# esologic/GANce

Measured on AMD Instinct MI355X. Metric: synthesized frames/sec at 1024x1024 config-f, higher is better.
Workload: dtype f32 (bf16x3 split operands, 6 terms, fp32 accumulate)

## Files before the change

gance_amd/csrc/upfir_split.hip:

```cpp

#include <hip/hip_runtime.h>

#include <algorithm>
#include <cstring>
#include <type_traits>

#include "kernels.h"

#ifndef GANCE_UPFIRS_ABLATE
#define GANCE_UPFIRS_ABLATE 0
#endif

namespace gance {

namespace {

typedef float f32x4 __attribute__((ext_vector_type(4)));
typedef float f32x2 __attribute__((ext_vector_type(2)));
typedef unsigned u32x4 __attribute__((ext_vector_type(4)));
typedef unsigned u32x2 __attribute__((ext_vector_type(2)));
typedef __bf16 bf16x8 __attribute__((ext_vector_type(8)));
typedef __bf16 bf16x2 __attribute__((ext_vector_type(2)));
typedef __attribute__((address_space(3))) void* lds_ptr_t;

constexpr int kBM = 16;
constexpr int kKC = 32;
constexpr int kSW = 64;
constexpr int kTH = 8;
constexpr int kRows = kTH + 1;
constexpr int kPlanes = 12;
constexpr int kPlaneStride = 80;
constexpr int kSlotUnits = kPlanes * kPlaneStride;
constexpr int kRing = 3;
constexpr int kHaloCols = 4;
constexpr int kHaloUnits = kRows * kHaloCols * kPlanes;
constexpr int kHaloTasks = kRows * kHaloCols * 4;
constexpr int kWeave = 2;
constexpr int kMinSegRows = 16;
constexpr int kDepth = 6;
constexpr int kCarryRows = 3;
constexpr int kPassCh = 4;
constexpr int kPassRows = 8;
constexpr float kSqrt2f = 1.4142135623730951f;
static_assert((2 * kRows) % kDepth == 0 && kDepth + 2 < kRows && kRows % kRing == 0, "ring slots and staging registers rotate with the unrolled rows of a chunk pair");

template <int NT>
struct Geo {
    static constexpr int kSW = 64 / NT;
    static constexpr int kBMB = kBM * NT;
    static constexpr int kTC = kSW / 16;
    static constexpr int kPW = 4 / NT;
    static constexpr int kTW = 2 * kSW + 4;
    static constexpr int kCG = kSW / 2;
    static constexpr int kRG = 64 / NT / kCG;
    static constexpr int kFR = kPassRows / kRG;
    static constexpr int kWin = kFR + 3;
    static constexpr int kCarryFloats = kBMB * kCarryRows * kTW;
    static constexpr int kStageFloats = kPassCh * NT * kPassRows * kTW;
    static constexpr int kNzPieces = 2 * kPassRows * 2 * kSW / 256;
    static constexpr int kWUnits = NT == 1 ? 27 * 64 : 0;
};

constexpr size_t kRingBytes = (size_t)kRing * kSlotUnits * 16;
constexpr size_t kHaloBytes = (size_t)2 * kHaloUnits * 16;
template <int NT>
constexpr size_t lds_bytes(int cin) {
    using G = Geo<NT>;
    return kRingBytes + kHaloBytes + (size_t)G::kWUnits * 16 +
           sizeof(float) * ((size_t)G::kStageFloats + G::kNzPieces * 256 + G::kCarryFloats + cin + 3 * G::kBMB);
}

__host__ __device__ constexpr int tap_cls(int t) { return t < 4 ? 0 : (t < 6 ? 1 : (t < 8 ? 2 : 3)); }
__host__ __device__ constexpr int tap_dy(int t) { return (t == 2 || t == 3 || t == 5) ? 1 : 0; }
__host__ __device__ constexpr int tap_dx(int t) { return (t == 1 || t == 3 || t == 7) ? 1 : 0; }

__device__ __forceinline__ void lds_barrier() {
    asm volatile("s_waitcnt lgkmcnt(0)" ::: "memory");
    __builtin_amdgcn_s_barrier();
    asm volatile("" ::: "memory");
}

__device__ __forceinline__ int fresh_lane() {
    int l;
    asm volatile("v_mbcnt_lo_u32_b32 %0, -1, 0\n\tv_mbcnt_hi_u32_b32 %0, -1, %0" : "=v"(l));
    return l;
}

__device__ __forceinline__ int ring_column(int P) {
    return ((P >> 2) & 3) | ((((P >> 4) ^ P) & 1) << 2) | (((P >> 1) & 1) << 3) | ((P & 1) << 4) | (P & 32);
}
constexpr int kEdgeColumn = 64;

__device__ __forceinline__ void split_pair(float a, float b, unsigned& p0, unsigned& p1, unsigned& p2) {
    auto pack = [](float lo, float hi) { return __builtin_bit_cast(unsigned, __builtin_convertvector(f32x2{lo, hi}, bf16x2)); };
    p0 = pack(a, b);
    const float ra = a - __builtin_bit_cast(float, p0 << 16), rb = b - __builtin_bit_cast(float, p0 & 0xffff0000u);
    p1 = pack(ra, rb);
    const float sa = ra - __builtin_bit_cast(float, p1 << 16), sb = rb - __builtin_bit_cast(float, p1 & 0xffff0000u);
    p2 = pack(sa, sb);
}

__device__ __forceinline__ void split_unit(const unsigned (&raw)[8], u32x4 (&part)[3]) {
    unsigned w[3][4];
    if (GANCE_UPFIRS_ABLATE & 1) {
#pragma unroll
        for (int q = 0; q < 3; ++q) part[q] = u32x4{raw[q], raw[q + 1], raw[q + 2], raw[q + 3]};
        return;
    }
#pragma unroll
    for (int e = 0; e < 4; ++e) split_pair(__builtin_bit_cast(float, raw[2 * e]), __builtin_bit_cast(float, raw[2 * e + 1]), w[0][e], w[1][e], w[2][e]);
#pragma unroll
    for (int q = 0; q < 3; ++q) part[q] = u32x4{w[q][0], w[q][1], w[q][2], w[q][3]};
}

}

template <int NT, bool kPre, bool kNoise>
__device__ __forceinline__ void upfirs_body(const UpFirArgs& p) {
    using G = Geo<NT>;
    constexpr int kSW = G::kSW, kBMB = G::kBMB, kTC = G::kTC, kPW = G::kPW, kTW = G::kTW, kCG = G::kCG, kRG = G::kRG, kFR = G::kFR,
                  kWin = G::kWin, kCarryFloats = G::kCarryFloats, kStageFloats = G::kStageFloats, kNzPieces = G::kNzPieces;
    extern __shared__ __attribute__((aligned(16))) unsigned char smem_raw[];
    u32x4* const ring = reinterpret_cast<u32x4*>(smem_raw);
    u32x4* const halo = ring + kRing * kSlotUnits;
    u32x4* const w_lds = halo + 2 * kHaloUnits;
    float* const stage = reinterpret_cast<float*>(w_lds + G::kWUnits);
    float* const nz_lds = stage + kStageFloats;
    float* const carry = nz_lds + kNzPieces * 256;
    float* const s_lds = carry + kCarryFloats;
    float* const d_lds = s_lds + (kPre ? 0 : p.Cin);
    float* const b_lds = d_lds + kBMB;
    float* const sn_lds = b_lds + kBMB;

    const int tid = threadIdx.x;
    const int wave = __builtin_amdgcn_readfirstlane(tid >> 6);
    const int lane = tid & 63;
    const int n16 = lane & 15, kg = lane >> 4;
    const int ct = NT == 1 ? 0 : wave / kTC, tc = NT == 1 ? wave : wave % kTC;

    int id;
    {
        const int v = blockIdx.x, nwg = p.total_blocks;
        const int q = nwg >> 3, r = nwg & 7, xcd = v & 7;
        id = (xcd < r ? xcd * (q + 1) : r * (q + 1) + (xcd - r) * q) + (v >> 3);
    }
    const int m_tile = id % p.m_tiles;
    id /= p.m_tiles;
    const int strip = id % p.strips;
    id /= p.strips;
    const int seg = id % p.segs;
    const int b = id / p.segs;
    const int m0 = m_tile * kBMB;
    const int X0 = strip * kSW;
    const int H = p.H, W = p.W;
    const int Hp = H + 2, Wp = W + 8;
    const int HpWp4 = Hp * Wp * 4;
    const int chunks = p.Cin / kKC;
    const int steps = H / kTH;
    const int s_begin = seg * (p.rows_per_seg / kTH), s_end = s_begin + p.rows_per_seg / kTH;
    const int s_first = seg > 0 ? s_begin - 1 : s_begin;

    const __amdgpu_buffer_rsrc_t x_rsrc =
        __builtin_amdgcn_make_buffer_rsrc((void*)(p.x + (size_t)b * p.x_b_stride), 0, p.Cin * Hp * Wp * 4, 0x00020000);
    const __amdgpu_buffer_rsrc_t w_rsrc = __builtin_amdgcn_make_buffer_rsrc(
        (void*)(reinterpret_cast<const unsigned char*>(p.w) + (size_t)(m_tile * NT + ct) * chunks * 27 * 1024), 0, chunks * 27 * 1024, 0x00020000);

    const int st_pair = lane >> 4, st_g = lane & 15;
    u32x4* const ring_w = ring + wave * kPlaneStride + ring_column(4 * st_g + st_pair);
    unsigned* const ring_wn = reinterpret_cast<unsigned*>(ring + wave * kPlaneStride + ring_column(NT == 2 ? 2 * st_g + (st_pair & 1) : st_g)) +
                              (NT == 2 ? 2 * (st_pair >> 1) : st_pair);
    const int m_pos = 16 * tc + n16;
    const u32x4* const ring_r0 = ring + kg * kPlaneStride + ring_column(m_pos);
    const u32x4* const ring_r1 = ring + kg * kPlaneStride + (m_pos > 0 ? ring_column(m_pos - 1) : kEdgeColumn);
    const bool edge_copy = wave == 3 && lane < kPlanes;
    const int e_unit = lane % kPlanes;
    u32x4* const ring_e = ring + (e_unit >> 2) * 4 * kPlaneStride + (e_unit & 3) * kPlaneStride + (edge_copy ? kEdgeColumn : 66 + wave);
    const u32x4* const halo_e = halo + e_unit;
    const u32x4* const halo_r = halo + ((n16 & 7) * kHaloCols + 2 * (n16 >> 3)) * kPlanes + kg;
    const u32x4* const halo_f = halo + ((kRows - 1) * kHaloCols + 2 * (n16 >> 3)) * kPlanes + kg;
    const int st_voff = (2 * st_pair * Hp * Wp + X0 + 4 + kPW * st_g) * 4;
    unsigned st[kDepth][8];
    auto stage_load = [&](unsigned(&dst)[8], int chunk, int brow, bool in_loop = false) {
        if ((GANCE_UPFIRS_ABLATE & 4) && in_loop) return;
        const int soff = ((chunk * kKC + wave * 8) * Hp + brow) * Wp * 4;
#pragma unroll
        for (int e = 0; e < 2; ++e) {
            if constexpr (kPW == 4) {
                const u32x4 q4 = __builtin_amdgcn_raw_buffer_load_b128(x_rsrc, st_voff, soff + e * HpWp4, 0);
#pragma unroll
                for (int c = 0; c < 4; ++c) dst[2 * c + e] = q4[c];
            } else if constexpr (kPW == 2) {
                const u32x2 q2 = __builtin_amdgcn_raw_buffer_load_b64(x_rsrc, st_voff, soff + e * HpWp4, 0);
                dst[e] = q2[0];
                dst[2 + e] = q2[1];
            } else {
                dst[e] = __builtin_amdgcn_raw_buffer_load_b32(x_rsrc, st_voff, soff + e * HpWp4, 0);
            }
        }
    };
    auto scale_pair = [&](unsigned(&raw)[8], int chunk) {
        if constexpr (!kPre) {
            const f32x2 s2 = *reinterpret_cast<const f32x2*>(s_lds + chunk * kKC + 8 * wave + 2 * st_pair);
#pragma unroll
            for (int c = 0; c < kPW; ++c) {
                raw[2 * c] = __builtin_bit_cast(unsigned, __builtin_bit_cast(float, raw[2 * c]) * s2[0]);
                raw[2 * c + 1] = __builtin_bit_cast(unsigned, __builtin_bit_cast(float, raw[2 * c + 1]) * s2[1]);
            }
        }
    };
    auto transpose_rows = [](u32x4& u) {
        auto a02 = __builtin_amdgcn_permlane32_swap(u[0], u[2], false, false);
        auto a13 = __builtin_amdgcn_permlane32_swap(u[1], u[3], false, false);
        auto b01 = __builtin_amdgcn_permlane16_swap(a02[0], a13[0], false, false);
        auto b23 = __builtin_amdgcn_permlane16_swap(a02[1], a13[1], false, false);
        u = u32x4{b01[0], b01[1], b23[0], b23[1]};
    };
    auto scale8 = [&](unsigned(&raw)[8], int chunk, int group) {
        if constexpr (!kPre) {
            const f32x4 s0 = *reinterpret_cast<const f32x4*>(s_lds + chunk * kKC + group * 8);
            const f32x4 s1 = *reinterpret_cast<const f32x4*>(s_lds + chunk * kKC + group * 8 + 4);
#pragma unroll
            for (int e = 0; e < 4; ++e) {
                raw[e] = __builtin_bit_cast(unsigned, __builtin_bit_cast(float, raw[e]) * s0[e]);
                raw[4 + e] = __builtin_bit_cast(unsigned, __builtin_bit_cast(float, raw[4 + e]) * s1[e]);
            }
        }
    };
    auto stage_store = [&](unsigned(&raw)[8], int slot, int chunk) {
        scale_pair(raw, chunk);
        if constexpr (NT == 1) {
            u32x4 part[3];
            split_unit(raw, part);
#pragma unroll
            for (int q = 0; q < 3; ++q) transpose_rows(part[q]);
#pragma unroll
            for (int q = 0; q < 3; ++q)
                if (!(GANCE_UPFIRS_ABLATE & 16)) ring_w[slot * kSlotUnits + q * 4 * kPlaneStride] = part[q];
        } else {
            unsigned w[3][kPW];
#pragma unroll
            for (int c = 0; c < kPW; ++c) split_pair(__builtin_bit_cast(float, raw[2 * c]), __builtin_bit_cast(float, raw[2 * c + 1]), w[0][c], w[1][c], w[2][c]);
#pragma unroll
            for (int q = 0; q < 3; ++q) {
                unsigned* const dst = ring_wn + 4 * (slot * kSlotUnits + q * 4 * kPlaneStride);
                if constexpr (NT == 2) {
                    const auto s = __builtin_amdgcn_permlane16_swap(w[q][0], w[q][1], false, false);
                    *reinterpret_cast<u32x2*>(dst) = u32x2{s[0], s[1]};
                } else {
                    *dst = w[q][0];
                }
            }
        }
    };
    auto edge_store = [&](int slot, int hbuf, int hrow) { if (!(GANCE_UPFIRS_ABLATE & 64)) ring_e[slot * kSlotUnits] = halo_e[hbuf * kHaloUnits + (hrow * kHaloCols + 1) * kPlanes]; };
    const int h_task = tid < kHaloTasks ? tid : tid - kHaloTasks;
    const int h_col = h_task & 3, h_kg = (h_task >> 2) & 3, h_row = h_task >> 4;
    const int h_voff = ((h_kg * 8 * Hp + h_row) * Wp + X0 + 2 + (h_col & 1) + (h_col >> 1) * (kSW + 1)) * 4;
    u32x4* const halo_w = halo + (h_row * kHaloCols + h_col) * kPlanes + h_kg;
    unsigned hraw[8];
    auto halo_load = [&](int step, int chunk) {
        const int soff = (chunk * kKC * Hp + kTH * step) * Wp * 4;
#pragma unroll
        for (int e = 0; e < 8; ++e) hraw[e] = __builtin_amdgcn_raw_buffer_load_b32(x_rsrc, h_voff, soff + e * HpWp4, 0);
    };
    auto halo_store = [&](int chunk, int buf) {
        scale8(hraw, chunk, h_kg);
        u32x4 part[3];
        split_unit(hraw, part);
#pragma unroll
        for (int q = 0; q < 3; ++q) halo_w[buf * kHaloUnits + q * 4] = part[q];
    };

    u32x4 A[9][3];
    const int a_voff = lane * 16;
    auto weights_dma = [&](int chunk) {
#pragma unroll
        for (int k = 0; k < 7; ++k)
            if (k < 6 || wave < 3)
                __builtin_amdgcn_raw_ptr_buffer_load_lds(w_rsrc, (lds_ptr_t)(w_lds + (wave + 4 * k) * 64), 16, lane * 16, (chunk * 27 + wave + 4 * k) * 1024, 0, 0);
    };
    const u32x4* const w_r = w_lds + lane;
    auto read_a3 = [&](int t, u32x4(&dst)[3]) {
#pragma unroll
        for (int q = 0; q < 3; ++q) dst[q] = w_r[(t * 3 + q) * 64];
    };
    auto load_a3 = [&](int chunk, int t, u32x4(&dst)[3]) {
#pragma unroll
        for (int q = 0; q < 3; ++q) dst[q] = __builtin_amdgcn_raw_buffer_load_b128(w_rsrc, a_voff, (chunk * 27 + t * 3 + q) * 1024, 0);
    };

    u32x4 Bf[2][2][3];
    auto load_b = [&](int slot, u32x4(&dst)[2][3]) {
#pragma unroll
        for (int q = 0; q < 3; ++q) {
            dst[0][q] = ring_r0[slot * kSlotUnits + q * 4 * kPlaneStride];
            dst[1][q] = ring_r1[slot * kSlotUnits + q * 4 * kPlaneStride];
        }
    };

    stage_load(st[0], 0, kTH * s_first + 0);
    stage_load(st[1], 0, kTH * s_first + 1);
    load_a3(0, 0, A[0]);
    halo_load(s_first, 0);
    if constexpr (!kPre)
        for (int i = tid; i < p.Cin; i += 256) s_lds[i] = p.s[(size_t)b * p.s_stride + i];
    if (tid < kBMB) {
        d_lds[tid] = p.d[(size_t)b * p.d_stride + m0 + tid];
        b_lds[tid] = p.bias[m0 + tid];
        sn_lds[tid] = p.s_next != nullptr ? p.s_next[(size_t)b * p.s_stride + m0 + tid] : 1.0f;
    }
    for (int i = tid; i < kCarryFloats; i += 256) carry[i] = 0.f;
    if constexpr (NT > 1)
        for (int i = tid; i < kPassCh * NT * kPassRows; i += 256) stage[i * kTW] = stage[i * kTW + 2 * kSW + 2] = stage[i * kTW + 2 * kSW + 3] = 0.f;
#pragma unroll
    for (int t = 1; t < 9; ++t) load_a3(0, t, A[t]);
    if constexpr (!kPre) lds_barrier();
    stage_store(st[0], 0, 0);
    stage_store(st[1], 1, 0);
    halo_store(0, 0);
#pragma unroll
    for (int r = 2; r < 2 + kDepth; ++r) stage_load(st[r % kDepth], 0, kTH * s_first + r);
    lds_barrier();
    edge_store(0, 0, 0);
    edge_store(1, 0, 1);
    lds_barrier();
    load_b(0, Bf[0]);

    const int OW = 2 * W, OWp = OW + 8;
    const long long oplane = (long long)(2 * H + 2) * OWp;
    const __amdgpu_buffer_rsrc_t o_rsrc = __builtin_amdgcn_make_buffer_rsrc(
        (void*)(p.out + ((size_t)b * p.Cout + m0) * oplane - 2 * OWp), 0, 0x7fffffff, 0x00020000);
    const __amdgpu_buffer_rsrc_t nz_rsrc = __builtin_amdgcn_make_buffer_rsrc(
        (void*)(kNoise ? p.noise + (size_t)b * p.noise_b_stride : nullptr), 0, kNoise ? (2 * H) * (2 * W) * 4 : 0, 0x00020000);
    const float ns2 = p.noise_strength * kSqrt2f;

    constexpr int kTerms[6][2] = {{2, 0}, {0, 2}, {1, 1}, {1, 0}, {0, 1}, {0, 0}};
    constexpr int kTapTurn[9] = {0, 4, 6, 8, 2, 5, 1, 7, 3};

#pragma unroll 1
    for (int si = s_first; si < s_end; ++si) {
        const int y0 = kTH * si;
        const bool last_step = si + 1 == steps;
        const bool priming = si < s_begin;
        f32x4 acc[kTH][4];
#pragma unroll
        for (int r = 0; r < kTH; ++r)
#pragma unroll
            for (int c = 0; c < 4; ++c) acc[r][c] = f32x4{0.f, 0.f, 0.f, 0.f};
        f32x4 accf[2] = {f32x4{0.f, 0.f, 0.f, 0.f}, f32x4{0.f, 0.f, 0.f, 0.f}};
        f32x4 acch[NT == 1 ? 1 : 2] = {}, acchf = f32x4{0.f, 0.f, 0.f, 0.f};

        auto run_chunk = [&](auto parity, const int chunk) {
            constexpr int ab = decltype(parity)::value;
            const int n_chunk = chunk + 1 < chunks ? chunk + 1 : 0;
            const int n_step = chunk + 1 < chunks ? si : (last_step ? si : si + 1);
#pragma unroll
            for (int j = 0; j < kRows; ++j) {
                const int cur = (j + ab) & 1;
                if (NT == 1 && j == 0) weights_dma(n_chunk);
                if (j == 0) halo_load(n_step, n_chunk);
                if (j == 4) halo_store(n_chunk, ab ^ 1);
                load_b((j + 1) % kRing, Bf[cur ^ 1]);
                edge_store((j + 2) % kRing, j + 2 < kRows ? ab : ab ^ 1, (j + 2) % kRows);
                stage_store(st[(kRows * ab + j + 2) % kDepth], (j + 2) % kRing, j + 2 < kRows ? chunk : n_chunk);
                stage_load(st[(kRows * ab + j + 2) % kDepth], j + 2 + kDepth < kRows ? chunk : n_chunk, kTH * (j + 2 + kDepth < kRows ? si : n_step) + (j + 2 + kDepth) % kRows, true);
                if (j + 1 < kRows) {
#pragma unroll
                    for (int term = 0; term < ((GANCE_UPFIRS_ABLATE & 8) ? 0 : 6); ++term)
#pragma unroll
                        for (int k = 0; k < 9; ++k) {
                            const int t = kTapTurn[k];
                            const int row = tap_dy(t) ? j : j - 1;
                            if (row < 0 || row >= kTH) continue;
                            acc[row][tap_cls(t)] = __builtin_amdgcn_mfma_f32_16x16x32_bf16(
                                __builtin_bit_cast(bf16x8, A[t][kTerms[term][1]]), __builtin_bit_cast(bf16x8, Bf[cur][tap_dx(t)][kTerms[term][0]]),
                                acc[row][tap_cls(t)], 0, 0, 0);
                        }
#pragma unroll
                    for (int i = 0; i < 54; ++i) {
                        if (i >= (j == 0 ? 18 : 54)) break;
                        __builtin_amdgcn_sched_group_barrier(0x008, 1, 0);
                        __builtin_amdgcn_sched_group_barrier(0x092, kWeave, 0);
                    }
                } else {
                    constexpr int kOrder[9] = {2, 3, 5, 0, 1, 4, 6, 7, 8};
#pragma unroll
                    for (int i = 0; i < 9; ++i) {
                        const int t = kOrder[i];
                        if (!tap_dy(t)) {
#pragma unroll
                            for (int term = 0; term < 6; ++term)
                                acc[kTH - 1][tap_cls(t)] = __builtin_amdgcn_mfma_f32_16x16x32_bf16(
                                    __builtin_bit_cast(bf16x8, A[t][kTerms[term][1]]), __builtin_bit_cast(bf16x8, Bf[cur][tap_dx(t)][kTerms[term][0]]),
                                    acc[kTH - 1][tap_cls(t)], 0, 0, 0);
                        } else if (last_step) {
#pragma unroll
                            for (int term = 0; term < 6; ++term)
                                accf[tap_cls(t)] = __builtin_amdgcn_mfma_f32_16x16x32_bf16(
                                    __builtin_bit_cast(bf16x8, A[t][kTerms[term][1]]), __builtin_bit_cast(bf16x8, Bf[cur][tap_dx(t)][kTerms[term][0]]),
                                    accf[tap_cls(t)], 0, 0, 0);
                        }
                        const int hc = NT == 1 ? 0 : tap_cls(t) >> 1;
                        const bool halo_mine = NT == 1 ? wave == tap_cls(t) : (tap_dx(t) && (tap_cls(t) & 1) == 0 && (kTC == 1 || tc == hc));
                        if (halo_mine && !(GANCE_UPFIRS_ABLATE & 64)) {
                            u32x4 hf[3];
#pragma unroll
                            for (int q = 0; q < 3; ++q) hf[q] = halo_r[ab * kHaloUnits + ((1 - tap_dy(t)) * kHaloCols + 1 - tap_dx(t)) * kPlanes + q * 4];
#pragma unroll
                            for (int term = 0; term < 6; ++term)
                                acch[hc] = __builtin_amdgcn_mfma_f32_16x16x32_bf16(__builtin_bit_cast(bf16x8, A[t][kTerms[term][1]]),
                                                                                    __builtin_bit_cast(bf16x8, hf[kTerms[term][0]]), acch[hc], 0, 0, 0);
                            if (last_step && tap_dy(t)) {
#pragma unroll
                                for (int q = 0; q < 3; ++q) hf[q] = halo_f[ab * kHaloUnits + (1 - tap_dx(t)) * kPlanes + q * 4];
#pragma unroll
                                for (int term = 0; term < 6; ++term)
                                    acchf = __builtin_amdgcn_mfma_f32_16x16x32_bf16(__builtin_bit_cast(bf16x8, A[t][kTerms[term][1]]),
                                                                                    __builtin_bit_cast(bf16x8, hf[kTerms[term][0]]), acchf, 0, 0, 0);
                            }
                        }
                        if constexpr (NT == 1) read_a3(t, A[t]);
                        else load_a3(n_chunk, t, A[t]);
                    }
                }
                if (NT == 1 && j == kRows - 2) asm volatile("s_waitcnt vmcnt(24)" ::: "memory");
                if (!(GANCE_UPFIRS_ABLATE & 32)) lds_barrier();
            }
        };
#pragma unroll 1
        for (int chunk = 0; chunk < chunks; chunk += 2) {
            run_chunk(std::integral_constant<int, 0>{}, chunk);
            run_chunk(std::integral_constant<int, 1>{}, chunk + 1);
        }

        const int elane = fresh_lane();
        const int en16 = elane & 15, eq4 = elane >> 4;
        const int dump_base = (4 * ct + eq4) * (kPassRows * kTW) + 32 * tc + 2 * en16 + 1;
        const int hpy = wave >> 1, hpx = wave & 1;
        const int fsub = NT == 1 ? 0 : elane / (64 / NT), flane = NT == 1 ? elane : elane % (64 / NT);
        const int fc = NT == 1 ? wave : wave * NT + fsub;
        const int fch = NT == 1 ? fc : 16 * (fc >> 2) + (fc & 3);
        const int cg = flane % kCG;
        const int rg = flane / kCG;
        const int o_voff = (int)((fch * oplane + (long long)(kFR * rg) * OWp + 4 * cg) * 4);

        auto run_passes = [&](auto flush_tag) {
            constexpr bool kFlush = decltype(flush_tag)::value;
            const int ys = kFlush ? H : y0;
            if (kNoise) {
#pragma unroll
                for (int i = 0; i < (kNzPieces + 3) / 4; ++i) {
                    if (kNzPieces % 4 != 0 && wave + 4 * i >= kNzPieces) break;
                    const int f = (wave + 4 * i) * 256 + 4 * elane;
                    const int row = f / (2 * kSW), col = f % (2 * kSW);
                    __builtin_amdgcn_raw_ptr_buffer_load_lds(nz_rsrc, (lds_ptr_t)(nz_lds + (wave + 4 * i) * 256), 16,
                                                             ((2 * ys - 2 + row) * OW + 2 * X0 + col) * 4, 0, 0, 0);
                }
                asm volatile("s_waitcnt vmcnt(0)" ::: "memory");
            }
            constexpr int kRowPasses = kFlush ? 1 : 2;
#pragma unroll
            for (int rw = 0; rw < kRowPasses; ++rw) {
                const int oy0 = 2 * (ys + 4 * rw) - 2;
                const int r_lo = max(0, -oy0);
                const int r_hi = priming ? 0 : min(kPassRows, 2 * H - oy0);
#pragma unroll
                for (int g = 0; g < 4; ++g) {
                    if constexpr (kFlush) {
#pragma unroll
                        for (int c = 0; c < 4; ++c) stage[dump_base + (c >> 1) * kTW + (c & 1)] = c < 2 ? accf[c][g] : 0.f;
                        if constexpr (NT == 1) {
                            if (en16 == 0 || en16 == 8) {
                                const int side = en16 >> 3;
                                if (hpy == 0 && (side == 1 || hpx == 1)) stage[eq4 * (kPassRows * kTW) + (side ? 2 * kSW + 1 + hpx : 0)] = acchf[g];
                                if (hpy == 1 && (side == 1 || hpx == 1)) stage[eq4 * (kPassRows * kTW) + kTW + (side ? 2 * kSW + 1 + hpx : 0)] = 0.f;
                            }
                        } else if (en16 == 8 && tc == 0) {
                            stage[(4 * ct + eq4) * (kPassRows * kTW) + 2 * kSW + 1] = acchf[g];
                            stage[(4 * ct + eq4) * (kPassRows * kTW) + kTW + 2 * kSW + 1] = 0.f;
                        }
                    } else {
#pragma unroll
                        for (int r4 = 0; r4 < 4; ++r4)
#pragma unroll
                            for (int c = 0; c < 4; ++c) stage[dump_base + (2 * r4 + (c >> 1)) * kTW + (c & 1)] = acc[4 * rw + r4][c][g];
                        const int row = en16 & 7, side = en16 >> 3;
                        if constexpr (NT == 1) {
                            if ((side == 1 || hpx == 1) && row / 4 == rw)
                                stage[eq4 * (kPassRows * kTW) + (2 * (row % 4) + hpy) * kTW + (side ? 2 * kSW + 1 + hpx : 0)] = acch[0][g];
                        } else if (side == 1 && row / 4 == rw) {
#pragma unroll
                            for (int h = 0; h < 2; ++h)
                                if (kTC == 1 || tc == h) stage[(4 * ct + eq4) * (kPassRows * kTW) + (2 * (row % 4) + h) * kTW + 2 * kSW + 1] = acch[h][g];
                        }
                    }
                    lds_barrier();

                    const int ch = 4 * g + fch;
                    const float dsc = d_lds[ch] * kSqrt2f;
                    const float kh0 = 0.25f * dsc, kh1 = 0.75f * dsc;
                    const float bias2 = b_lds[ch] * kSqrt2f;
                    const float lr6 = 0.6f * sn_lds[ch], lr4 = 0.4f * sn_lds[ch];
                    const float* const win_lo = carry + ch * (kCarryRows * kTW) + (kFR * rg) * kTW + 4 * cg;
                    const float* const win_hi = stage + fc * (kPassRows * kTW) + (kFR * rg - kCarryRows) * kTW + 4 * cg;
                    f32x4 ta[kWin], tb[kWin];
#pragma unroll
                    for (int i = 0; i < kWin; ++i) {
                        const float* const rowp = (i < kCarryRows && kFR * rg + i < kCarryRows ? win_lo : win_hi) + i * kTW;
                        ta[i] = *reinterpret_cast<const f32x4*>(rowp);
                        tb[i] = *reinterpret_cast<const f32x4*>(rowp + 4);
                    }
                    {
                        const int o_soff = (int)((4 * g * oplane + (long long)(oy0 + 3) * OWp + 2 * X0 + 4) * 4);
#pragma unroll
                        for (int r = 0; r < kFR; ++r) {
                            const int rr = kFR * rg + r;
                            if (rr >= r_lo && rr < r_hi) {
                                f32x2 tv[4];
#pragma unroll
                                for (int c2 = 0; c2 < 4; ++c2) {
                                    auto pair = [&](int i) { return c2 < 2 ? f32x2{ta[i][2 * c2], ta[i][2 * c2 + 1]} : f32x2{tb[i][2 * c2 - 4], tb[i][2 * c2 - 3]}; };
                                    tv[c2] = 0.25f * pair(r) + 0.75f * pair(r + 1) + 0.75f * pair(r + 2) + 0.25f * pair(r + 3);
                                }
                                const float t[7] = {tv[0][0], tv[0][1], tv[1][0], tv[1][1], tv[2][0], tv[2][1], tv[3][0]};
                                f32x4 v;
#pragma unroll
                                for (int o = 0; o < 4; ++o) v[o] = fmaf(kh0, t[o + 3], fmaf(kh1, t[o + 2], fmaf(kh1, t[o + 1], fmaf(kh0, t[o], bias2))));
                                if (kNoise) v += ns2 * *reinterpret_cast<const f32x4*>(nz_lds + (kPassRows * rw + rr) * (2 * kSW) + 4 * cg);
#pragma unroll
                                for (int o = 0; o < 4; ++o) v[o] = fmaf(lr6, v[o], lr4 * __builtin_fabsf(v[o]));
                                if (!(GANCE_UPFIRS_ABLATE & 128)) __builtin_amdgcn_raw_buffer_store_b128(__builtin_bit_cast(u32x4, v), o_rsrc, o_voff, o_soff + r * OWp * 4, 0);
                                else asm volatile("" ::"v"(v));
                            }
                        }
                    }
                    lds_barrier();
                    if (!kFlush && rg == kRG - 1) {
                        float* const carry_w = carry + ch * (kCarryRows * kTW) + 4 * cg;
#pragma unroll
                        for (int i = 0; i < 3; ++i) {
                            *reinterpret_cast<f32x4*>(carry_w + i * kTW) = ta[kWin - 3 + i];
                            if (cg == kCG - 1) *reinterpret_cast<f32x4*>(carry_w + i * kTW + 4) = tb[kWin - 3 + i];
                        }
                    }
                }
            }
        };
        if (GANCE_UPFIRS_ABLATE & 2) {
            float sum = acch[0][0] + acchf[0] + accf[0][0] + accf[1][0];
#pragma unroll
            for (int r = 0; r < kTH; ++r)
#pragma unroll
                for (int c = 0; c < 4; ++c) sum += acc[r][c][0] + acc[r][c][3];
            if (sum == 12345.678f) p.out[tid] = sum;
            continue;
        }
        run_passes(std::false_type{});
        if (last_step) {
            lds_barrier();
            run_passes(std::true_type{});
        }
    }
}

bool upfirs_supported(int cin, int cout, int H, int W) {
    return H == W && W % kSW == 0 && H % kTH == 0 && cin % (2 * kKC) == 0 && cout % kBM == 0 && cin <= 512;
}

bool upfirs_narrow_supported(int cin, int cout, int H, int W) {
    return H == W && (W == 32 || W == 16) && H % kTH == 0 && cin % (2 * kKC) == 0 && cout % (kBM * (kSW / W)) == 0 && cin <= 512;
}

size_t upfirs_weight_floats(int cin, int cout) { return (size_t)(cout / kBM) * (cin / kKC) * 27 * 256; }

static unsigned short bf16_rne_host(float x) {
    unsigned u;
    std::memcpy(&u, &x, 4);
    u += 0x7fffu + ((u >> 16) & 1u);
    return (unsigned short)(u >> 16);
}
static float bf16_value_host(unsigned short h) {
    const unsigned u = (unsigned)h << 16;
    float f;
    std::memcpy(&f, &u, 4);
    return f;
}

void upfirs_arrange_weights(const float* w_in, int cin, int cout, const int* up_tap_weight, float* w_out) {
    unsigned short* const out = reinterpret_cast<unsigned short*>(w_out);
    const int m_tiles = cout / kBM, chunks = cin / kKC;
    for (int mt = 0; mt < m_tiles; ++mt)
        for (int ch = 0; ch < chunks; ++ch)
            for (int t = 0; t < 9; ++t)
                for (int k = 0; k < kKC; ++k)
                    for (int m = 0; m < kBM; ++m) {
                        const int channel = 4 * (m & 3) + (m >> 2);
                        const float v = w_in[((size_t)up_tap_weight[t] * cin + ch * kKC + k) * cout + mt * kBM + channel];
                        unsigned short part[3];
                        part[0] = bf16_rne_host(v);
                        const float r1 = v - bf16_value_host(part[0]);
                        part[1] = bf16_rne_host(r1);
                        part[2] = bf16_rne_host(r1 - bf16_value_host(part[1]));
                        for (int q = 0; q < 3; ++q)
                            out[((((((size_t)mt * chunks + ch) * 9 + t) * 3 + q) * 4 + k / 8) * 16 + m) * 8 + k % 8] = part[q];
                    }
}

void upfirs_plan(int B, int cout, int H, int W, int num_cus, UpFirArgs* a) {
    a->step_rows = kTH;
    if (W < kSW) {
        a->m_tiles = cout / (kBM * (kSW / W));
        a->strips = 1;
        a->segs = 1;
        a->rows_per_seg = H;
        a->total_blocks = B * a->m_tiles;
        return;
    }
    a->m_tiles = cout / kBM;
    a->strips = W / kSW;
    int segs = 1;
    const int base = B * a->m_tiles * a->strips;
    long long best = (long long)((base + num_cus - 1) / num_cus) * H;
    for (int n = 2; H / n >= kMinSegRows && (H / n) % kTH == 0 && base * (n / 2) < num_cus; n *= 2) {
        const long long cost = (long long)((base * n + num_cus - 1) / num_cus) * (H / n + kTH);
        if (cost < best) best = cost, segs = n;
    }
    a->segs = segs;
    a->rows_per_seg = H / segs;
    a->total_blocks = base * segs;
}

__global__ __launch_bounds__(256, 1) void upfirs_fused_kernel(const UpFirArgs p) { upfirs_body<1, false, false>(p); }
__global__ __launch_bounds__(256, 1) void upfirs_fused_noise_kernel(const UpFirArgs p) { upfirs_body<1, false, true>(p); }
__global__ __launch_bounds__(256, 1) void upfirs_fused_pre_kernel(const UpFirArgs p) { upfirs_body<1, true, false>(p); }
__global__ __launch_bounds__(256, 1) void upfirs_fused_pre_noise_kernel(const UpFirArgs p) { upfirs_body<1, true, true>(p); }
__global__ __launch_bounds__(256, 1) void upfirs_w32_fused_kernel(const UpFirArgs p) { upfirs_body<2, false, false>(p); }
__global__ __launch_bounds__(256, 1) void upfirs_w32_fused_noise_kernel(const UpFirArgs p) { upfirs_body<2, false, true>(p); }
__global__ __launch_bounds__(256, 1) void upfirs_w32_fused_pre_kernel(const UpFirArgs p) { upfirs_body<2, true, false>(p); }
__global__ __launch_bounds__(256, 1) void upfirs_w32_fused_pre_noise_kernel(const UpFirArgs p) { upfirs_body<2, true, true>(p); }
__global__ __launch_bounds__(256, 1) void upfirs_w16_fused_kernel(const UpFirArgs p) { upfirs_body<4, false, false>(p); }
__global__ __launch_bounds__(256, 1) void upfirs_w16_fused_noise_kernel(const UpFirArgs p) { upfirs_body<4, false, true>(p); }
__global__ __launch_bounds__(256, 1) void upfirs_w16_fused_pre_kernel(const UpFirArgs p) { upfirs_body<4, true, false>(p); }
__global__ __launch_bounds__(256, 1) void upfirs_w16_fused_pre_noise_kernel(const UpFirArgs p) { upfirs_body<4, true, true>(p); }

hipError_t launch_upfir_split(const UpFirArgs& args, hipStream_t stream) {
    using Kernel = void (*)(const UpFirArgs);
    static const Kernel kernels[3][4] = {
        {upfirs_fused_kernel, upfirs_fused_noise_kernel, upfirs_fused_pre_kernel, upfirs_fused_pre_noise_kernel},
        {upfirs_w32_fused_kernel, upfirs_w32_fused_noise_kernel, upfirs_w32_fused_pre_kernel, upfirs_w32_fused_pre_noise_kernel},
        {upfirs_w16_fused_kernel, upfirs_w16_fused_noise_kernel, upfirs_w16_fused_pre_kernel, upfirs_w16_fused_pre_noise_kernel}};
    static size_t (*const lds_of[3])(int) = {lds_bytes<1>, lds_bytes<2>, lds_bytes<4>};
    static PerDeviceInt ready;
    int unused = 0;
    const hipError_t e = ready.get(
        [&](int, int* value) {
            *value = 1;
            for (int gi = 0; gi < 3; ++gi)
                for (int i = 0; i < 4; ++i) {
                    const hipError_t err = hipFuncSetAttribute(reinterpret_cast<const void*>(kernels[gi][i]), hipFuncAttributeMaxDynamicSharedMemorySize,
                                                               (int)lds_of[gi](i >= 2 ? 0 : 512));
                    if (err != hipSuccess) return err;
                }
            return hipSuccess;
        },
        &unused);
    if (e != hipSuccess) return e;
    const int gi = args.W % kSW == 0 ? 0 : (args.W == 32 ? 1 : 2);
    const bool narrow = gi != 0;
    if (!(narrow ? upfirs_narrow_supported(args.Cin, args.Cout, args.H, args.W) : upfirs_supported(args.Cin, args.Cout, args.H, args.W)) || args.segs < 1 ||
        args.rows_per_seg * args.segs != args.H || args.rows_per_seg % kTH != 0 || args.total_blocks != args.B * args.m_tiles * args.strips * args.segs ||
        (narrow && (args.segs != 1 || args.strips != 1 || args.m_tiles * kBM * (kSW / args.W) != args.Cout)))
        return hipErrorInvalidValue;
    const int pre = args.input_prescaled ? 1 : 0, noise = args.noise != nullptr ? 1 : 0;
    hipLaunchKernelGGL(kernels[gi][2 * pre + noise], dim3(args.total_blocks), dim3(256), lds_of[gi](pre ? 0 : args.Cin), stream, args);
    return hipGetLastError();
}

}
```

Measured before the change: 1486.

## Apply vertical FIR in registers before staging for single-tile upfir epilogue

For the NT==1 path, the epilogue now computes the vertical 4-tap upsampling FIR directly from accumulator registers, with per-lane carry rows kept in LDS. Only the vertically filtered rows go to a double-buffered stage, and halo columns are handled through a small ring buffer. This replaces staging raw accumulators, so the shared-memory read window per row shrinks and every other barrier can be skipped. The cost is a larger carry region, two stage buffers, and more complex indexing that risks correctness at boundaries and flush steps.

Result: no change. 1501, median of 6 (+1.0%).

```diff
diff --git a/gance_amd/csrc/upfir_split.hip b/gance_amd/csrc/upfir_split.hip
--- a/gance_amd/csrc/upfir_split.hip
+++ b/gance_amd/csrc/upfir_split.hip
@@ -55,8 +55,11 @@
     static constexpr int kRG = 64 / NT / kCG;
     static constexpr int kFR = kPassRows / kRG;
     static constexpr int kWin = kFR + 3;
-    static constexpr int kCarryFloats = kBMB * kCarryRows * kTW;
     static constexpr int kStageFloats = kPassCh * NT * kPassRows * kTW;
+    static constexpr int kStageBufs = NT == 1 ? 2 : 1;
+    static constexpr int kLaneCarryFloats = 2 * kCarryRows * 256 * 4;
+    static constexpr int kHaloRing = 32, kHaloTCols = 3;
+    static constexpr int kCarryFloats = NT == 1 ? kLaneCarryFloats + kBM * kHaloRing * kHaloTCols : kBMB * kCarryRows * kTW;
     static constexpr int kNzPieces = 2 * kPassRows * 2 * kSW / 256;
     static constexpr int kWUnits = NT == 1 ? 27 * 64 : 0;
 };
@@ -67,8 +70,9 @@
 constexpr size_t lds_bytes(int cin) {
     using G = Geo<NT>;
     return kRingBytes + kHaloBytes + (size_t)G::kWUnits * 16 +
-           sizeof(float) * ((size_t)G::kStageFloats + G::kNzPieces * 256 + G::kCarryFloats + cin + 3 * G::kBMB);
-}
+           sizeof(float) * ((size_t)G::kStageBufs * G::kStageFloats + G::kNzPieces * 256 + G::kCarryFloats + cin + 3 * G::kBMB);
+}
+static_assert(lds_bytes<1>(512) <= 160 * 1024 && lds_bytes<2>(512) <= 160 * 1024 && lds_bytes<4>(512) <= 160 * 1024, "a CU's LDS");
 
 __host__ __device__ constexpr int tap_cls(int t) { return t < 4 ? 0 : (t < 6 ? 1 : (t < 8 ? 2 : 3)); }
 __host__ __device__ constexpr int tap_dy(int t) { return (t == 2 || t == 3 || t == 5) ? 1 : 0; }
@@ -111,6 +115,17 @@
     for (int e = 0; e < 4; ++e) split_pair(__builtin_bit_cast(float, raw[2 * e]), __builtin_bit_cast(float, raw[2 * e + 1]), w[0][e], w[1][e], w[2][e]);
 #pragma unroll
     for (int q = 0; q < 3; ++q) part[q] = u32x4{w[q][0], w[q][1], w[q][2], w[q][3]};
+}
+
+__device__ __forceinline__ float vfir(int rr, float a, float b, float c, float d) {
+    const float ab = rr % 4 == 0 ? __builtin_fmaf(0.75f, b, 0.25f * a) : __builtin_fmaf(0.25f, a, 0.75f * b);
+    return __builtin_fmaf(0.25f, d, __builtin_fmaf(0.75f, c, ab));
+}
+
+__device__ __forceinline__ float acc_read(float a) {
+    float v;
+    asm volatile("v_accvgpr_read_b32 %0, %1" : "=v"(v) : "a"(a));
+    return v;
 }
 
 }
@@ -125,7 +140,7 @@
     u32x4* const halo = ring + kRing * kSlotUnits;
     u32x4* const w_lds = halo + 2 * kHaloUnits;
     float* const stage = reinterpret_cast<float*>(w_lds + G::kWUnits);
-    float* const nz_lds = stage + kStageFloats;
+    float* const nz_lds = stage + G::kStageBufs * kStageFloats;
     float* const carry = nz_lds + kNzPieces * 256;
     float* const s_lds = carry + kCarryFloats;
     float* const d_lds = s_lds + (kPre ? 0 : p.Cin);
@@ -433,16 +448,42 @@
             run_chunk(std::integral_constant<int, 1>{}, chunk + 1);
         }
 
+        if (GANCE_UPFIRS_ABLATE & 2) {
+            float sum = acch[0][0] + acchf[0] + accf[0][0] + accf[1][0];
+#pragma unroll
+            for (int r = 0; r < kTH; ++r)
+#pragma unroll
+                for (int c = 0; c < 4; ++c) sum += acc[r][c][0] + acc[r][c][3];
+            if (sum == 12345.678f) p.out[tid] = sum;
+            continue;
+        }
+        if constexpr (NT == 1) {
         const int elane = fresh_lane();
+        asm volatile("s_nop 15\n\ts_nop 15" ::: "memory");
         const int en16 = elane & 15, eq4 = elane >> 4;
-        const int dump_base = (4 * ct + eq4) * (kPassRows * kTW) + 32 * tc + 2 * en16 + 1;
         const int hpy = wave >> 1, hpx = wave & 1;
-        const int fsub = NT == 1 ? 0 : elane / (64 / NT), flane = NT == 1 ? elane : elane % (64 / NT);
-        const int fc = NT == 1 ? wave : wave * NT + fsub;
-        const int fch = NT == 1 ? fc : 16 * (fc >> 2) + (fc & 3);
-        const int cg = flane % kCG;
-        const int rg = flane / kCG;
-        const int o_voff = (int)((fch * oplane + (long long)(kFR * rg) * OWp + 4 * cg) * 4);
+        f32x4* const lcarry = reinterpret_cast<f32x4*>(carry) + 64 * wave + elane;
+        float* const halo_t = carry + G::kLaneCarryFloats;
+        constexpr int kHCh = G::kHaloRing * G::kHaloTCols;
+        const int k0 = ((si - s_first) & 1) * 16;
+        const int dump_base = eq4 * (kPassRows * kTW) + 32 * tc + 2 * en16 + 1;
+        const int cg = elane % kCG, rg = elane / kCG;
+        const int o_voff = (int)((wave * oplane + (long long)(kFR * rg) * OWp + 4 * cg) * 4);
+        const int hv_r = elane / G::kHaloTCols, hv_c = elane % G::kHaloTCols;
+
+        {
+            const int row = en16 & 7, side = en16 >> 3;
+            if (side == 1 || hpx == 1) {
+                float* const h = halo_t + (eq4 * G::kHaloRing + k0 + 2 * row + hpy) * G::kHaloTCols + (side ? 1 + hpx : 0);
+#pragma unroll
+                for (int g = 0; g < 4; ++g) h[4 * g * kHCh] = acch[0][g];
+                if (last_step && row == 0) {
+                    float* const hf = halo_t + (eq4 * G::kHaloRing + (k0 ^ 16) + hpy) * G::kHaloTCols + (side ? 1 + hpx : 0);
+#pragma unroll
+                    for (int g = 0; g < 4; ++g) hf[4 * g * kHCh] = hpy == 0 ? acchf[g] : 0.f;
+                }
+            }
+        }
 
         auto run_passes = [&](auto flush_tag) {
             constexpr bool kFlush = decltype(flush_tag)::value;
@@ -458,6 +499,107 @@
                 }
                 asm volatile("s_waitcnt vmcnt(0)" ::: "memory");
             }
+            lds_barrier();
+            constexpr int kRowPasses = kFlush ? 1 : 2;
+            constexpr int kURows = kFlush ? 2 : kPassRows;
+#pragma unroll
+            for (int rw = 0; rw < kRowPasses; ++rw) {
+                const int oy0 = 2 * (ys + 4 * rw) - 2;
+                const int r_lo = max(0, -oy0);
+                const int r_hi = min(kPassRows, 2 * H - oy0);
+#pragma unroll
+                for (int g = 0; g < 4; ++g) {
+                    float* const sbuf = stage + ((4 * rw + g) & 1) * kStageFloats;
+                    float w[kURows + kCarryRows][2];
+#pragma unroll
+                    for (int R = 0; R < kURows + kCarryRows; ++R)
+#pragma unroll
+                        for (int px = 0; px < 2; ++px) {
+                            const int j = (kFlush ? 2 * kTH : kPassRows * rw) + R - kCarryRows;
+                            if (j < 0) w[R][px] = reinterpret_cast<const float*>(lcarry + (2 * R + px) * 256)[g];
+                            else if (j < 2 * kTH) w[R][px] = acc_read(acc[j >> 1][2 * (j & 1) + px][g]);
+                            else w[R][px] = j == 2 * kTH ? acc_read(accf[px][g]) : 0.f;
+                        }
+#pragma unroll
+                    for (int rr = 0; rr < kURows; ++rr)
+#pragma unroll
+                        for (int px = 0; px < 2; ++px) sbuf[dump_base + rr * kTW + px] = vfir(rr, w[rr][px], w[rr + 1][px], w[rr + 2][px], w[rr + 3][px]);
+                    if (elane < kPassRows * G::kHaloTCols) {
+                        const float* const h = halo_t + (4 * g + wave) * kHCh + hv_c;
+                        const int r0 = (kFlush ? k0 : (k0 ^ 16) + kPassRows * rw) + 16 - kCarryRows + hv_r;
+                        float t[4];
+#pragma unroll
+                        for (int i = 0; i < 4; ++i) t[i] = h[((r0 + i) & (G::kHaloRing - 1)) * G::kHaloTCols];
+                        const float u0 = vfir(0, t[0], t[1], t[2], t[3]), u1 = vfir(1, t[0], t[1], t[2], t[3]);
+                        sbuf[wave * (kPassRows * kTW) + hv_r * kTW + (hv_c ? 2 * kSW + hv_c : 0)] = hv_r % kFR == 0 ? u0 : u1;
+                    }
+                    lds_barrier();
+
+                    const int ch = 4 * g + wave;
+                    const float dsc = d_lds[ch] * kSqrt2f;
+                    const float kh0 = 0.25f * dsc, kh1 = 0.75f * dsc;
+                    const float bias2 = b_lds[ch] * kSqrt2f;
+                    const float lr6 = 0.6f * sn_lds[ch], lr4 = 0.4f * sn_lds[ch];
+                    const float* const urow = sbuf + wave * (kPassRows * kTW) + (kFR * rg) * kTW + 4 * cg;
+                    f32x4 ua[kFR], ub[kFR];
+#pragma unroll
+                    for (int r = 0; r < kFR; ++r) {
+                        ua[r] = *reinterpret_cast<const f32x4*>(urow + r * kTW);
+                        ub[r] = *reinterpret_cast<const f32x4*>(urow + r * kTW + 4);
+                    }
+                    const int o_soff = (int)((4 * g * oplane + (long long)(oy0 + 3) * OWp + 2 * X0 + 4) * 4);
+#pragma unroll
+                    for (int r = 0; r < kFR; ++r) {
+                        const int rr = kFR * rg + r;
+                        if (rr >= r_lo && rr < r_hi) {
+                            const float t[7] = {ua[r][0], ua[r][1], ua[r][2], ua[r][3], ub[r][0], ub[r][1], ub[r][2]};
+                            f32x4 v;
+#pragma unroll
+                            for (int o = 0; o < 4; ++o) v[o] = fmaf(kh0, t[o + 3], fmaf(kh1, t[o + 2], fmaf(kh1, t[o + 1], fmaf(kh0, t[o], bias2))));
+                            if (kNoise) v += ns2 * *reinterpret_cast<const f32x4*>(nz_lds + (kPassRows * rw + rr) * (2 * kSW) + 4 * cg);
+#pragma unroll
+                            for (int o = 0; o < 4; ++o) v[o] = fmaf(lr6, v[o], lr4 * __builtin_fabsf(v[o]));
+                            if (!(GANCE_UPFIRS_ABLATE & 128)) __builtin_amdgcn_raw_buffer_store_b128(__builtin_bit_cast(u32x4, v), o_rsrc, o_voff, o_soff + r * OWp * 4, 0);
+                            else asm volatile("" ::"v"(v));
+                        }
+                    }
+                }
+            }
+        };
+        if (!priming) run_passes(std::false_type{});
+#pragma unroll
+        for (int i = 0; i < kCarryRows; ++i)
+#pragma unroll
+            for (int px = 0; px < 2; ++px) lcarry[(2 * i + px) * 256] = acc[(2 * kTH - kCarryRows + i) >> 1][2 * ((2 * kTH - kCarryRows + i) & 1) + px];
+        if (last_step) {
+            lds_barrier();
+            run_passes(std::true_type{});
+        }
+        } else {
+        const int elane = fresh_lane();
+        const int en16 = elane & 15, eq4 = elane >> 4;
+        const int dump_base = (4 * ct + eq4) * (kPassRows * kTW) + 32 * tc + 2 * en16 + 1;
+        const int fsub = elane / (64 / NT), flane = elane % (64 / NT);
+        const int fc = wave * NT + fsub;
+        const int fch = 16 * (fc >> 2) + (fc & 3);
+        const int cg = flane % kCG;
+        const int rg = flane / kCG;
+        const int o_voff = (int)((fch * oplane + (long long)(kFR * rg) * OWp + 4 * cg) * 4);
+
+        auto run_passes = [&](auto flush_tag) {
+            constexpr bool kFlush = decltype(flush_tag)::value;
+            const int ys = kFlush ? H : y0;
+            if (kNoise) {
+#pragma unroll
+                for (int i = 0; i < (kNzPieces + 3) / 4; ++i) {
+                    if (kNzPieces % 4 != 0 && wave + 4 * i >= kNzPieces) break;
+                    const int f = (wave + 4 * i) * 256 + 4 * elane;
+                    const int row = f / (2 * kSW), col = f % (2 * kSW);
+                    __builtin_amdgcn_raw_ptr_buffer_load_lds(nz_rsrc, (lds_ptr_t)(nz_lds + (wave + 4 * i) * 256), 16,
+                                                             ((2 * ys - 2 + row) * OW + 2 * X0 + col) * 4, 0, 0, 0);
+                }
+                asm volatile("s_waitcnt vmcnt(0)" ::: "memory");
+            }
             constexpr int kRowPasses = kFlush ? 1 : 2;
 #pragma unroll
             for (int rw = 0; rw < kRowPasses; ++rw) {
@@ -469,13 +611,7 @@
                     if constexpr (kFlush) {
 #pragma unroll
                         for (int c = 0; c < 4; ++c) stage[dump_base + (c >> 1) * kTW + (c & 1)] = c < 2 ? accf[c][g] : 0.f;
-                        if constexpr (NT == 1) {
-                            if (en16 == 0 || en16 == 8) {
-                                const int side = en16 >> 3;
-                                if (hpy == 0 && (side == 1 || hpx == 1)) stage[eq4 * (kPassRows * kTW) + (side ? 2 * kSW + 1 + hpx : 0)] = acchf[g];
-                                if (hpy == 1 && (side == 1 || hpx == 1)) stage[eq4 * (kPassRows * kTW) + kTW + (side ? 2 * kSW + 1 + hpx : 0)] = 0.f;
-                            }
-                        } else if (en16 == 8 && tc == 0) {
+                        if (en16 == 8 && tc == 0) {
                             stage[(4 * ct + eq4) * (kPassRows * kTW) + 2 * kSW + 1] = acchf[g];
                             stage[(4 * ct + eq4) * (kPassRows * kTW) + kTW + 2 * kSW + 1] = 0.f;
                         }
@@ -485,10 +621,7 @@
 #pragma unroll
                             for (int c = 0; c < 4; ++c) stage[dump_base + (2 * r4 + (c >> 1)) * kTW + (c & 1)] = acc[4 * rw + r4][c][g];
                         const int row = en16 & 7, side = en16 >> 3;
-                        if constexpr (NT == 1) {
-                            if ((side == 1 || hpx == 1) && row / 4 == rw)
-                                stage[eq4 * (kPassRows * kTW) + (2 * (row % 4) + hpy) * kTW + (side ? 2 * kSW + 1 + hpx : 0)] = acch[0][g];
-                        } else if (side == 1 && row / 4 == rw) {
+                        if (side == 1 && row / 4 == rw) {
 #pragma unroll
                             for (int h = 0; h < 2; ++h)
                                 if (kTC == 1 || tc == h) stage[(4 * ct + eq4) * (kPassRows * kTW) + (2 * (row % 4) + h) * kTW + 2 * kSW + 1] = acch[h][g];
@@ -546,19 +679,11 @@
                 }
             }
         };
-        if (GANCE_UPFIRS_ABLATE & 2) {
-            float sum = acch[0][0] + acchf[0] + accf[0][0] + accf[1][0];
-#pragma unroll
-            for (int r = 0; r < kTH; ++r)
-#pragma unroll
-                for (int c = 0; c < 4; ++c) sum += acc[r][c][0] + acc[r][c][3];
-            if (sum == 12345.678f) p.out[tid] = sum;
-            continue;
-        }
         run_passes(std::false_type{});
         if (last_step) {
             lds_barrier();
             run_passes(std::true_type{});
+        }
         }
     }
 }
```
